# surrealdb/surrealdb

Measured on NVIDIA H100. Metric: KNN queries/sec @recall@10=1.0 (exact brute force), higher is better.
Workload: dtype s8 screen + f64 exact

## Files before the change

### surrealdb_b200/csrc/api.cu

```cuda
#include <cmath>

#include <algorithm>
#include <chrono>

#include "internal.cuh"

namespace sdb {

static thread_local char g_err[1024] = "";
void set_error(const char* fmt, ...) {
  va_list ap;
  va_start(ap, fmt);
  vsnprintf(g_err, sizeof(g_err), fmt, ap);
  va_end(ap);
}


static uint32_t pass_ratio(uint32_t nq) {
  static int env = -1;
  if (env < 0) {
    env = 0;
    if (const char* e = getenv("SDB_PASS_RATIO")) {
      const int v = atoi(e);
      if (v >= 2 && v <= 64) env = v;
// ... 698 lines not shown
      }
    }
  }
  if (lane == 0) out_count[q] = n_out;
}

sdb_status topk_merge_launch(Ctx* ctx, uint32_t n_lists, uint32_t nq, uint32_t k, const uint64_t* d_rows,
                             const double* d_dist, const uint32_t* d_counts, uint64_t stride_rows, uint64_t stride_dist,
                             uint64_t stride_counts, uint64_t* d_out_rows, double* d_out_dist, uint32_t* d_out_count,
                             cudaStream_t st) {
  if (!stride_rows) stride_rows = (uint64_t)nq * k;
  if (!stride_dist) stride_dist = (uint64_t)nq * k;
  if (!stride_counts) stride_counts = nq;
  if (n_lists <= 32) {
    topk_kway_merge_kernel<<<(nq + 3) / 4, 128, 0, st>>>(n_lists, nq, k, d_rows, d_dist, d_counts, stride_rows, stride_dist,
                                                       stride_counts, d_out_rows, d_out_dist, d_out_count);
    count_launch(ctx);
    SDB_CUDA(cudaGetLastError());
    return SDB_OK;
  }
  uint32_t p2 = 1;
  while (p2 < n_lists * k) p2 <<= 1;
  const size_t smem = (size_t)p2 * 24;
  if (smem > 200 * 1024) {
    set_error("merge of %u lists x k=%u exceeds the shared-memory sorter", n_lists, k);
    return SDB_EUNSUPPORTED;
  }
  const uint32_t threads = p2 >= 1024 ? 1024 : (p2 < 64 ? 64 : p2);
  topk_merge_kernel<<<nq, threads, smem, st>>>(n_lists, nq, k, d_rows, d_dist, d_counts, stride_rows, stride_dist,
                                               stride_counts, d_out_rows, d_out_dist, d_out_count);
  count_launch(ctx);
  SDB_CUDA(cudaGetLastError());
  return SDB_OK;
}

}

using namespace sdb;

extern "C" {

const char* sdb_last_error(void) { return g_err; }
const char* sdb_version(void) { return "sdbgpu 0.1.0 (sm_90a)"; }

sdb_status sdb_ctx_create(int device, sdb_ctx** out) {
  if (!out) return SDB_EINVAL;
  *out = nullptr;
  int n = 0;
  cudaError_t e = cudaGetDeviceCount(&n);
  if (e != cudaSuccess || n == 0) {
    set_error("no CUDA device available (%s); this library has no CPU fallback", cudaGetErrorString(e));
    return SDB_ECUDA;
  }
  if (device < 0 || device >= n) {
    set_error("device %d out of range (0..%d)", device, n - 1);
    return SDB_EINVAL;
  }
  cudaDeviceProp prop;
  SDB_CUDA(cudaGetDeviceProperties(&prop, device));
  if (prop.major != 9 || prop.minor != 0) {
    set_error("device %d is sm_%d%d; this library ships sm_90a code only", device, prop.major, prop.minor);
    return SDB_ECUDA;
  }
  SDB_CUDA(cudaSetDevice(device));
  sdb_ctx* c = new sdb_ctx();
  c->device = device;
  c->sm_count = prop.multiProcessorCount;
  {
    int least = 0, greatest = 0;
    if (cudaDeviceGetStreamPriorityRange(&least, &greatest) == cudaSuccess) c->prio_high = greatest;
  }
  SDB_CUDA(cudaStreamCreateWithFlags(&c->stream, cudaStreamNonBlocking));
  SDB_CUDA(cudaStreamCreateWithFlags(&c->stream2, cudaStreamNonBlocking));
  SDB_CUDA(cudaStreamCreateWithFlags(&c->copy_stream, cudaStreamNonBlocking));
  {
    int* hc = nullptr;
    SDB_CUDA(cudaHostAlloc(&hc, sizeof(int), cudaHostAllocMapped));
    *hc = 0;
    c->h_cancel = hc;
    SDB_CUDA(cudaMalloc(&c->d_cancel, sizeof(int)));
    SDB_CUDA(cudaMemset(c->d_cancel, 0, sizeof(int)));
    SDB_CUDA(cudaStreamCreateWithFlags(&c->cancel_stream, cudaStreamNonBlocking));
  }
  SDB_TRY(screen_tc_init_device());
  SDB_TRY(candidates_init_device());
  SDB_TRY(exact_init_device());
  SDB_CUDA(cudaFuncSetAttribute(topk_merge_kernel, cudaFuncAttributeMaxDynamicSharedMemorySize, 200 * 1024));
  {
    cudaMemPool_t pool;
    if (cudaDeviceGetDefaultMemPool(&pool, device) == cudaSuccess) {
      uint64_t thr = ~0ull;
      cudaMemPoolSetAttribute(pool, cudaMemPoolAttrReleaseThreshold, &thr);
    }
  }
  *out = c;
  return SDB_OK;
}
void sdb_ctx_destroy(sdb_ctx* c) {
  if (!c) return;
  cudaSetDevice(c->device);
  comm_destroy(c);
  if (c->stream) cudaStreamDestroy(c->stream);
  if (c->stream2) cudaStreamDestroy(c->stream2);
  if (c->copy_stream) cudaStreamDestroy(c->copy_stream);
  if (c->h_stage) cudaFreeHost(c->h_stage);
  if (c->h_cancel) cudaFreeHost((void*)c->h_cancel);
  if (c->d_cancel) cudaFree(c->d_cancel);
  if (c->cancel_stream) cudaStreamDestroy(c->cancel_stream);
  delete c;
}
static void push_cancel_word(sdb_ctx* c) {
  if (!c->d_cancel || !c->cancel_stream) return;
  if (cudaSetDevice(c->device) != cudaSuccess) return;
  cudaMemcpyAsync(c->d_cancel, (const void*)c->h_cancel, sizeof(int), cudaMemcpyHostToDevice, c->cancel_stream);
  cudaStreamSynchronize(c->cancel_stream);
}
void sdb_ctx_cancel(sdb_ctx* c) {
  if (!c || !c->h_cancel) return;
  *c->h_cancel = 1;
  push_cancel_word(c);
}
void sdb_ctx_cancel_reset(sdb_ctx* c) {
  if (!c || !c->h_cancel) return;
  *c->h_cancel = 0;
  push_cancel_word(c);
}
uint64_t sdb_ctx_kernel_launches(const sdb_ctx* c) { return c ? c->launches : 0; }
void* sdb_ctx_stream(const sdb_ctx* c) { return c ? (void*)c->stream : nullptr; }
void* sdb_pinned_alloc(size_t bytes) {
  void* p = nullptr;
  if (cudaHostAlloc(&p, bytes, cudaHostAllocDefault) != cudaSuccess) {
    set_error("cudaHostAlloc(%zu) failed", bytes);
    return nullptr;
  }
  return p;
}
void sdb_pinned_free(void* p) {
  if (p) cudaFreeHost(p);
}
void sdb_free(void* p) { free(p); }

sdb_status sdb_corpus_create(sdb_ctx* ctx, uint32_t dim, sdb_dtype dt, sdb_metric m, uint64_t cap, sdb_corpus** out) {
  if (!ctx || !out || dim == 0 || dim > 65535 || cap == 0 || cap >= 0xFFFFFFF0ull) {
    set_error("sdb_corpus_create: bad argument (dim 1..65535, 0 < capacity < 2^32)");
    return SDB_EINVAL;
  }
  const bool screenable = m == SDB_COSINE || m == SDB_EUCLIDEAN;
  if ((int)m < 0 || (int)m > (int)SDB_PEARSON) {
    set_error("unknown metric %d", (int)m);
    return SDB_EINVAL;
  }
  if (dt != SDB_F32 && dt != SDB_F64) return SDB_EINVAL;
  SDB_CUDA(cudaSetDevice(ctx->device));
  sdb_corpus* c = new sdb_corpus();
  c->ctx = ctx;
  c->dim = dim;
  c->dim_pad = (dim + 63) / 64 * 64;
  c->dim_pad8 = (dim + 127) / 128 * 128;
  c->dtype = dt;
  c->metric = m;
  c->cap = cap;
  const size_t esz = dt == SDB_F32 ? 4 : 8;
  const uint64_t cap_pad = (cap + TILE_ROWS - 1) / TILE_ROWS * TILE_ROWS;
  cudaError_t e = cudaMalloc(&c->d_rows, esz * cap * dim);
  if (e == cudaSuccess) e = cudaMalloc(&c->d_mag, sizeof(double) * cap);
  if (e == cudaSuccess) e = cudaMalloc(&c->d_snorm, sizeof(float) * cap_pad);
  if (e == cudaSuccess && dt == SDB_F32 && screenable) e = cudaMalloc(&c->d_bf16, sizeof(__nv_bfloat16) * cap_pad * c->dim_pad);
// ... 564 lines not shown
```

### surrealdb_b200/csrc/internal.cuh

```cuda
#pragma once
#include <cuda_bf16.h>
#include <cuda_runtime.h>

#include <cstdarg>
#include <cstdint>
#include <cstdio>
#include <cstdlib>
#include <cstring>
#include <mutex>
#include <vector>

#include "../../include/sdbgpu.h"

namespace sdb {

void set_error(const char* fmt, ...);

#define SDB_CUDA(call)                                                                      \
  do {                                                                                      \
    cudaError_t e__ = (call);                                                               \
    if (e__ != cudaSuccess) {                                                               \
      ::sdb::set_error("%s:%d: %s -> %s", __FILE__, __LINE__, #call, cudaGetErrorString(e__)); \
      return SDB_ECUDA;                                                                     \
    }                                                                                       \
// ... 15 lines not shown
#else
  memcpy(&b, &d, 8);
#endif
  return b;
}
__host__ __device__ inline uint64_t dist_key(double d) {
  uint64_t b = f64_bits(d);
  if ((b << 1) == 0) b = 0;
  return (b >> 63) ? ~b : (b | 0x8000000000000000ull);
}
__host__ __device__ inline uint32_t f32_key(float f) {
  uint32_t b;
#ifdef __CUDA_ARCH__
  asm volatile("mov.b32 %0, %1;" : "=r"(b) : "f"(f));
#else
  memcpy(&b, &f, 4);
#endif
  return (b >> 31) ? ~b : (b | 0x80000000u);
}

constexpr uint32_t HIST_BINS = 256;
constexpr uint32_t PROBE_TILES_MAX = 64;
constexpr uint32_t PROBE_STRIDE = PROBE_TILES_MAX * 8;
struct HistParam {
  float lo;
  float inv_w0;
  float w0;
  float margin;
};
__host__ __device__ inline uint32_t hist_bin(const HistParam& p, float score) {
  float t = (score - p.lo) * p.inv_w0 + 1.0f;
  t = t >= 1.0f ? t : 1.0f;
  uint32_t b;
#ifdef __CUDA_ARCH__
  b = (__float_as_uint(t) - 0x3F800000u) >> 19;
#else
  uint32_t u;
  memcpy(&u, &t, 4);
  b = (u - 0x3F800000u) >> 19;
#endif
  return b < HIST_BINS - 1 ? b : HIST_BINS - 1;
}
__host__ __device__ inline double hist_edge(const HistParam& p, uint32_t b) {
  const uint32_t u = 0x3F800000u + (b << 19);
  float t;
#ifdef __CUDA_ARCH__
  t = __uint_as_float(u);
#else
  memcpy(&t, &u, 4);
#endif
  return (double)p.lo + (double)p.w0 * ((double)t - 1.0);
}

struct PassDesc {
  uint32_t stride;
  uint32_t excl;
  uint32_t count;
  uint32_t perm;
};
__host__ __device__ inline uint32_t pass_tile(const PassDesc& p, uint32_t w) {
  if (p.perm) w = (uint32_t)(((uint64_t)w * p.perm) % p.count);
  uint32_t i = p.excl ? (w / (p.excl - 1)) * p.excl + (w % (p.excl - 1)) + 1 : w;
  return i * p.stride;
}

struct Comm;

struct Ctx {
  int device = 0;
  int sm_count = 132;
  cudaStream_t stream = nullptr;
  cudaStream_t stream2 = nullptr;
  cudaStream_t copy_stream = nullptr;
  uint64_t launches = 0;
  std::mutex mu;
  void* encode_tiled = nullptr;
  void* h_stage = nullptr;
  size_t h_stage_bytes = 0;
  Comm* comm = nullptr;
  volatile int* h_cancel = nullptr;
  int* d_cancel = nullptr;
  cudaStream_t cancel_stream = nullptr;
  int prio_high = 0;
  cudaEvent_t trace_epoch = nullptr;
  double trace_host0 = 0.0;
};
inline bool ctx_cancelled(const Ctx* ctx) { return ctx->h_cancel && *ctx->h_cancel != 0; }

sdb_status screen_tc_init_device();
sdb_status candidates_init_device();
sdb_status exact_init_device();
void comm_destroy(Ctx* ctx);
void comm_corpus_released(struct Corpus* c);
int comm_size(const Ctx* ctx);
int comm_rank(const Ctx* ctx);
sdb_status comm_allreduce_sum(Ctx* ctx, void* d_buf, size_t count, int elem_bytes, cudaStream_t st);

struct Cand {
  float score;
  uint32_t row;
};

struct Ticket {
  bool busy = false;
  uint32_t id = 0;
  const double* d_queries = nullptr;
  uint32_t nq = 0, k = 0;
  uint64_t row_base = 0;
  uint64_t *d_out_rows = nullptr, *h_out_rows = nullptr;
  double *d_out_dist = nullptr, *h_out_dist = nullptr;
  uint32_t *d_out_count = nullptr, *h_out_count = nullptr;
  const volatile int* cancel = nullptr;
  cudaStream_t stream = nullptr;
  int set = 0;
  int screen = 0;
  uint32_t rung = 0, n_rungs = 0, n_batch_rungs = 0, n_repaired = 0;
  uint32_t n_passes = 0;
  uint64_t launches0 = 0;
  cudaEvent_t ev_begin = nullptr, ev_screen0 = nullptr, ev_screen1 = nullptr, ev_end = nullptr;
  uint32_t* h_flags = nullptr;
  uint32_t* h_qflags = nullptr;
  uint32_t* h_stat = nullptr;
  uint32_t h_cap = 0;
  double* d_in_q = nullptr;
  uint64_t* d_res_rows = nullptr;
  double* d_res_dist = nullptr;
  uint32_t* d_res_count = nullptr;
  size_t in_cap = 0, res_cap = 0, res_cap_q = 0;
  cudaEvent_t ev_h2d = nullptr, ev_out = nullptr;
  cudaEvent_t ev_main = nullptr;
  bool wait_h2d = false;
  std::vector<std::pair<const char*, cudaEvent_t>> trace;
};
constexpr int N_TICKETS = 4;
bool trace_enabled();
void trace_mark(Ctx* ctx, Ticket& t, const char* name, cudaStream_t st);
void trace_dump(Ctx* ctx, Ticket& t);
void trace_host(Ctx* ctx, uint32_t ticket, const char* name);

struct Scratch {
  uint32_t sc_nq = 0, sc_cap = 0;
  double* d_q64 = nullptr;
  float* d_q32 = nullptr;
  __nv_bfloat16* d_qbf16 = nullptr;
  double* d_qmag = nullptr;
  uint32_t* d_qflags = nullptr;
  float* d_qbferr = nullptr;
  int8_t* d_q8 = nullptr;
  float* d_q8scale = nullptr;
  float* d_q8err = nullptr;
  Cand* d_sub = nullptr;
  uint32_t* d_sub_cnt = nullptr;
  uint32_t sub_slots = 0, sub_cap = 0, last_slots = 0;
  float* d_bscale = nullptr;
  float* d_beps = nullptr;
  float* d_margin = nullptr;
  float* d_margin2 = nullptr;
  float* d_beps2 = nullptr;
  float* d_tau2 = nullptr;
  float* d_qlow = nullptr;
  float* d_qcap = nullptr;
  HistParam* d_hparam = nullptr;
  uint32_t* d_hist = nullptr;
  float* d_probe = nullptr;
  float* d_tau = nullptr;
  Cand* d_cand = nullptr;
  uint32_t* d_cand_cnt = nullptr;
  uint32_t* d_flags = nullptr;
  uint32_t* d_stat = nullptr;
  uint64_t* d_rr_key = nullptr;
  double* d_rr_dist = nullptr;
  uint32_t* d_rr_row = nullptr;
// ... 110 lines not shown
```

### surrealdb_b200/csrc/screen_tc.cu

```cuda
#include <cuda.h>

#include <type_traits>

#include "internal.cuh"

namespace sdb {

namespace tc {
constexpr uint32_t BLOCK_M = 128;
constexpr uint32_t BLOCK_N = 256;
constexpr uint32_t BLOCK_K = 64;
constexpr uint32_t WG_M = 64;
constexpr uint32_t STAGES = 4;
constexpr uint32_t A_BYTES = BLOCK_M * BLOCK_K * 2;
constexpr uint32_t B_BYTES = BLOCK_N * BLOCK_K * 2;
constexpr uint32_t STAGE_BYTES = A_BYTES + B_BYTES;
constexpr uint32_t CONS_WARPS = 8;
constexpr uint32_t PROD_WARP = CONS_WARPS;
constexpr uint32_t THREADS = (CONS_WARPS + 2) * 32;
constexpr uint32_t MAX_MBLOCKS = 16;
constexpr uint32_t SUBCAP = 16;
constexpr uint32_t SMEM_BYTES = STAGES * STAGE_BYTES + 2 * BLOCK_N * 4 + 256 + MAX_MBLOCKS * 256 * 4 + 1024;
static_assert(BLOCK_N == TILE_ROWS, "screen tile must match the pass schedule tile");
static_assert(SMEM_BYTES <= 227 * 1024, "screen CTA must fit the shared memory of one SM");

__device__ __forceinline__ uint32_t smem_u32(const void* p) { return (uint32_t)__cvta_generic_to_shared(p); }

__device__ __forceinline__ uint32_t item_mb(uint32_t w, uint32_t n_mb) { return (w % n_mb + w / n_mb) % n_mb; }

__device__ __forceinline__ void mbar_init(uint32_t bar, uint32_t count) {
  asm volatile("mbarrier.init.shared::cta.b64 [%0], %1;" ::"r"(bar), "r"(count) : "memory");
}
__device__ __forceinline__ void mbar_expect_tx(uint32_t bar, uint32_t bytes) {
  asm volatile("mbarrier.arrive.expect_tx.shared::cta.b64 _, [%0], %1;" ::"r"(bar), "r"(bytes) : "memory");
}
__device__ __forceinline__ void mbar_arrive(uint32_t bar) {
  asm volatile("mbarrier.arrive.shared::cta.b64 _, [%0];" ::"r"(bar) : "memory");
}
__device__ __forceinline__ void mbar_wait(uint32_t bar, uint32_t parity) {
  uint32_t ok;
  do {
    asm volatile(
        "{\n\t.reg .pred p;\n\t"
        "mbarrier.try_wait.parity.shared::cta.b64 p, [%1], %2;\n\t"
        "selp.u32 %0, 1, 0, p;\n\t}"
        : "=r"(ok)
        : "r"(bar), "r"(parity)
        : "memory");
  } while (!ok);
}
__device__ __forceinline__ void tma_load_2d(uint32_t dst, const CUtensorMap* map, uint32_t c0, uint32_t c1, uint32_t bar) {
  asm volatile(
      "cp.async.bulk.tensor.2d.shared::cluster.global.tile.mbarrier::complete_tx::bytes [%0], [%1, {%2, %3}], [%4];"
      ::"r"(dst), "l"(map), "r"(c0), "r"(c1), "r"(bar)
      : "memory");
}

#define SDB_WG_REGS                                                                                   \
  "{%0, %1, %2, %3, %4, %5, %6, %7, %8, %9, %10, %11, %12, %13, %14, %15, "                           \
  "%16, %17, %18, %19, %20, %21, %22, %23, %24, %25, %26, %27, %28, %29, %30, %31, "                  \
  "%32, %33, %34, %35, %36, %37, %38, %39, %40, %41, %42, %43, %44, %45, %46, %47, "                  \
  "%48, %49, %50, %51, %52, %53, %54, %55, %56, %57, %58, %59, %60, %61, %62, %63, "                  \
  "%64, %65, %66, %67, %68, %69, %70, %71, %72, %73, %74, %75, %76, %77, %78, %79, "                  \
  "%80, %81, %82, %83, %84, %85, %86, %87, %88, %89, %90, %91, %92, %93, %94, %95, "                  \
  "%96, %97, %98, %99, %100, %101, %102, %103, %104, %105, %106, %107, %108, %109, %110, %111, "      \
  "%112, %113, %114, %115, %116, %117, %118, %119, %120, %121, %122, %123, %124, %125, %126, %127}"
#define SDB_WG8(C, i) C(d[i]), C(d[i + 1]), C(d[i + 2]), C(d[i + 3]), C(d[i + 4]), C(d[i + 5]), C(d[i + 6]), C(d[i + 7])
#define SDB_WG128(C)                                                                                     \
  SDB_WG8(C, 0), SDB_WG8(C, 8), SDB_WG8(C, 16), SDB_WG8(C, 24), SDB_WG8(C, 32), SDB_WG8(C, 40), SDB_WG8(C, 48), \
      SDB_WG8(C, 56), SDB_WG8(C, 64), SDB_WG8(C, 72), SDB_WG8(C, 80), SDB_WG8(C, 88), SDB_WG8(C, 96),             \
      SDB_WG8(C, 104), SDB_WG8(C, 112), SDB_WG8(C, 120)

__device__ __forceinline__ void wgmma_bf16(float (&d)[128], uint64_t a_desc, uint64_t b_desc, uint32_t acc) {
  asm volatile(
      "{\n\t.reg .pred p;\n\t"
      "setp.ne.b32 p, %130, 0;\n\t"
      "wgmma.mma_async.sync.aligned.m64n256k16.f32.bf16.bf16 " SDB_WG_REGS ", %128, %129, p, 1, 1, 0, 0;\n\t}"
      : SDB_WG128("+f")
      : "l"(a_desc), "l"(b_desc), "r"(acc));
}
__device__ __forceinline__ void wgmma_i8(uint32_t (&d)[128], uint64_t a_desc, uint64_t b_desc, uint32_t acc) {
  asm volatile(
      "{\n\t.reg .pred p;\n\t"
      "setp.ne.b32 p, %130, 0;\n\t"
      "wgmma.mma_async.sync.aligned.m64n256k32.s32.s8.s8 " SDB_WG_REGS ", %128, %129, p;\n\t}"
      : SDB_WG128("+r")
      : "l"(a_desc), "l"(b_desc), "r"(acc));
}
__device__ __forceinline__ void acc_fence(float (&d)[128]) {
#pragma unroll
  for (int i = 0; i < 128; i++) asm volatile("" : "+f"(d[i])::"memory");
}
__device__ __forceinline__ void acc_fence(uint32_t (&d)[128]) {
#pragma unroll
  for (int i = 0; i < 128; i++) asm volatile("" : "+r"(d[i])::"memory");
}
#undef SDB_WG128
#undef SDB_WG8
#undef SDB_WG_REGS
__device__ __forceinline__ void wgmma_fence() { asm volatile("wgmma.fence.sync.aligned;" ::: "memory"); }
__device__ __forceinline__ void wgmma_commit() { asm volatile("wgmma.commit_group.sync.aligned;" ::: "memory"); }
template <int N>
__device__ __forceinline__ void wgmma_wait() {
  asm volatile("wgmma.wait_group.sync.aligned %0;" ::"n"(N) : "memory");
}
__device__ __forceinline__ uint64_t make_desc(uint32_t saddr) {
  uint64_t d = 0;
  d |= (uint64_t)((saddr >> 4) & 0x3FFF);
  d |= (uint64_t)1 << 16;
  d |= (uint64_t)(1024 >> 4) << 32;
  d |= (uint64_t)1 << 62;
  return d;
}

template <typename Acc>
__device__ __forceinline__ Acc acc_at(const Acc (&acc)[128], int i, int t) {
  return acc[4 * (t >> 1) + 2 * i + (t & 1)];
}
__device__ __forceinline__ uint32_t fragment_col(int t, uint32_t col_l) { return 8 * (t >> 1) + col_l + (t & 1); }
template <typename Acc>
__device__ __forceinline__ Acc acc_at_dyn(const Acc (&acc)[128], int i, int t) {
  Acc v = acc[2 * i];
#pragma unroll
  for (int u = 1; u < 64; u++) v = u == t ? acc_at(acc, i, u) : v;
  return v;
}


template <int MODE>
__device__ __forceinline__ void append_survivor(float score, uint32_t q, uint32_t row, uint32_t col, uint32_t row0,
                                                float2 hpv, uint32_t* s_cnt_mb, Cand* __restrict__ cand,
                                                uint32_t* __restrict__ cand_cnt, uint32_t cap, Cand* __restrict__ sub,
                                                uint32_t* hist) {
  const uint32_t half = col >> 7;
  const uint32_t pos = atomicAdd(s_cnt_mb + half * BLOCK_M + row, 1u);
  const uint2 cd = make_uint2(__float_as_uint(score), row0 + col);
  const uint32_t n_slots = gridDim.x * 2;
  if (pos < SUBCAP) {
    *reinterpret_cast<uint2*>(sub + ((size_t)q * n_slots + blockIdx.x * 2 + half) * SUBCAP + pos) = cd;
  } else {
    const uint32_t p2 = atomicAdd(cand_cnt + q, 1u);
    if (p2 < cap) *reinterpret_cast<uint2*>(cand + (size_t)q * cap + p2) = cd;
  }
  if (MODE == 2) {
    HistParam hp;
    hp.lo = hpv.x;
    hp.inv_w0 = hpv.y;
    hp.w0 = 0.f;
    hp.margin = 0.f;
    atomicAdd(hist + (size_t)q * HIST_BINS + hist_bin(hp, score), 1u);
  }
}

template <bool COSINE, bool INT8, int MODE>
__global__ void __launch_bounds__(THREADS, 1)
screen_tc_kernel(const __grid_constant__ CUtensorMap map_a, const __grid_constant__ CUtensorMap map_b,
                 const float* __restrict__ snorm, uint32_t k_blocks, uint32_t n_mblocks, uint32_t nq,
                 PassDesc pass, float* tau, Cand* __restrict__ cand,
                 uint32_t* __restrict__ cand_cnt, uint32_t cap, Cand* __restrict__ sub, uint32_t* __restrict__ sub_cnt,
                 uint32_t k, const HistParam* __restrict__ hparam, uint32_t* hist, float* __restrict__ probe,
                 uint32_t probe_stride, uint32_t sleep_min_ns, uint32_t sleep_max_ns) {
  extern __shared__ uint8_t smem_raw[];
  uint8_t* smem = reinterpret_cast<uint8_t*>((reinterpret_cast<uintptr_t>(smem_raw) + 1023) & ~uintptr_t(1023));
  uint8_t* smem_a = smem;
  uint8_t* smem_b = smem + STAGES * A_BYTES;
  float* s_snorm = reinterpret_cast<float*>(smem + STAGES * STAGE_BYTES);
  uint64_t* bars = reinterpret_cast<uint64_t*>(s_snorm + 2 * BLOCK_N);
  uint64_t* full_bar = bars;
  uint64_t* empty_bar = bars + STAGES;
  uint32_t* s_done = reinterpret_cast<uint32_t*>(bars + 2 * STAGES);
  uint32_t* s_cnt = reinterpret_cast<uint32_t*>(reinterpret_cast<uint8_t*>(bars) + 256);

  const uint32_t warp = threadIdx.x >> 5, lane = threadIdx.x & 31;
  const uint32_t n_items = pass.count * n_mblocks;

  if (threadIdx.x == 0) {
    asm volatile("prefetch.tensormap [%0];" ::"l"(&map_a) : "memory");
    asm volatile("prefetch.tensormap [%0];" ::"l"(&map_b) : "memory");
    for (uint32_t s = 0; s < STAGES; s++) {
      mbar_init(smem_u32(&full_bar[s]), 1);
      mbar_init(smem_u32(&empty_bar[s]), CONS_WARPS);
    }
    asm volatile("fence.mbarrier_init.release.cluster;" ::: "memory");
    *s_done = 0;
  }
  for (uint32_t i = threadIdx.x; i < n_mblocks * 256; i += blockDim.x) s_cnt[i] = 0;
  __syncthreads();

  if (warp == PROD_WARP) {
    if (lane == 0) {
      uint32_t it = 0;
      for (uint32_t w = blockIdx.x; w < n_items; w += gridDim.x) {
        const uint32_t tile = pass_tile(pass, w / n_mblocks);
        const uint32_t mb = item_mb(w, n_mblocks);
        for (uint32_t kb = 0; kb < k_blocks; kb++, it++) {
          const uint32_t s = it % STAGES, ph = (it / STAGES) & 1;
          mbar_wait(smem_u32(&empty_bar[s]), ph ^ 1);
          const uint32_t fb = smem_u32(&full_bar[s]);
          mbar_expect_tx(fb, STAGE_BYTES);
          tma_load_2d(smem_u32(smem_a + s * A_BYTES), &map_a, kb * (INT8 ? 2 * BLOCK_K : BLOCK_K), mb * BLOCK_M, fb);
          tma_load_2d(smem_u32(smem_b + s * B_BYTES), &map_b, kb * (INT8 ? 2 * BLOCK_K : BLOCK_K), tile * BLOCK_N, fb);
        }
      }
    }
    __syncwarp();
  } else if (warp < CONS_WARPS) {
    const uint32_t ct = threadIdx.x;
    const uint32_t g = warp >> 2;
    const uint32_t row_base = g * WG_M + (warp & 3) * 16 + (lane >> 2);
    const uint32_t col_l = 2 * (lane & 3);
    constexpr bool pass0 = MODE == 0;
    using Acc = typename std::conditional<INT8, uint32_t, float>::type;
    Acc acc[128];
    uint32_t it = 0, j = 0;
    for (uint32_t w = blockIdx.x; w < n_items; w += gridDim.x, j++) {
      const uint32_t tidx = w / n_mblocks;
      const uint32_t tile = pass_tile(pass, tidx);
      const uint32_t mb = item_mb(w, n_mblocks);
      const uint32_t row0 = tile * BLOCK_N;
      float my_tau[2];
      float2 my_hp[2];
#pragma unroll
      for (int i = 0; i < 2; i++) {
        const uint32_t q = mb * BLOCK_M + row_base + 8 * i;
        my_tau[i] = __int_as_float(0x7f800000);
        my_hp[i] = make_float2(0.f, 0.f);
        if (q < nq) {
          my_tau[i] = __ldcg(tau + q);
          if (MODE == 2) my_hp[i] = __ldg(reinterpret_cast<const float2*>(hparam + q));
        }
      }
      float* sn = s_snorm + (j & 1) * BLOCK_N;
      if (!INT8 || MODE == 3) {
        sn[ct] = __ldg(snorm + row0 + ct);
        asm volatile("bar.sync 1, 256;" ::: "memory");
      }

      const uint32_t a_off = g * (WG_M * 128);
      for (uint32_t kb = 0; kb < k_blocks; kb++, it++) {
        const uint32_t s = it % STAGES, ph = (it / STAGES) & 1;
        mbar_wait(smem_u32(&full_bar[s]), ph);
        const uint64_t da = make_desc(smem_u32(smem_a + s * A_BYTES + a_off));
        const uint64_t db = make_desc(smem_u32(smem_b + s * B_BYTES));
        wgmma_fence();
        acc_fence(acc);
#pragma unroll
        for (uint32_t kk = 0; kk < 4; kk++) {
          if constexpr (INT8) wgmma_i8(acc, da + 2 * kk, db + 2 * kk, (kb | kk) != 0);
          else wgmma_bf16(acc, da + 2 * kk, db + 2 * kk, (kb | kk) != 0);
        }
        wgmma_commit();
        acc_fence(acc);
        if (kb > 0) {
          wgmma_wait<1>();
          if (lane == 0) mbar_arrive(smem_u32(&empty_bar[(it - 1) % STAGES]));
        }
      }
      wgmma_wait<0>();
      acc_fence(acc);
      if (lane == 0) mbar_arrive(smem_u32(&empty_bar[(it - 1) % STAGES]));

      if constexpr (!INT8) {
#pragma unroll
        for (int jj = 0; jj < 32; jj++) {
          const float2 n2 = *reinterpret_cast<const float2*>(sn + 8 * jj + col_l);
#pragma unroll
          for (int i = 0; i < 2; i++) {
            float& a0 = acc[4 * jj + 2 * i];
            float& a1 = acc[4 * jj + 2 * i + 1];
            a0 = COSINE ? a0 * n2.x : fmaf(2.f, a0, -n2.x);
            a1 = COSINE ? a1 * n2.y : fmaf(2.f, a1, -n2.y);
          }
        }
      }
#pragma unroll
      for (int i = 0; i < 2; i++) {
        const uint32_t row = row_base + 8 * i;
        const uint32_t q = mb * BLOCK_M + row;
        if (MODE == 3) {
#pragma unroll
          for (int h = 0; h < 8; h++) {
            float m = __int_as_float(0xff800000);
#pragma unroll
            for (int jj = 4 * h; jj < 4 * h + 4; jj++) {
#pragma unroll
              for (int c = 0; c < 2; c++) {
                if constexpr (INT8) {
                  const float snv = sn[8 * jj + col_l + c];
                  if (snv == snv) m = fmaxf(m, __int2float_rd((int)acc[4 * jj + 2 * i + c]));
                } else {
                  m = fmaxf(m, acc[4 * jj + 2 * i + c]);
                }
              }
            }
            m = fmaxf(m, __shfl_xor_sync(0xffffffffu, m, 1));
            m = fmaxf(m, __shfl_xor_sync(0xffffffffu, m, 2));
            if ((lane & 3) == 0 && q < nq) probe[(size_t)q * probe_stride + tidx * 8 + h] = m;
          }
        } else if (pass0) {
          if (q < nq) {
            Cand* my_cand = cand + (size_t)q * cap + (size_t)tidx * BLOCK_N;
#pragma unroll
            for (int jj = 0; jj < 32; jj++) {
              const uint32_t col = 8 * jj + col_l;
              float s0, s1;
              if constexpr (INT8) {
                s0 = __int2float_rn((int)acc[4 * jj + 2 * i]);
                s1 = __int2float_rn((int)acc[4 * jj + 2 * i + 1]);
              } else {
                s0 = acc[4 * jj + 2 * i];
                s1 = acc[4 * jj + 2 * i + 1];
              }
              *reinterpret_cast<uint2*>(my_cand + col) = make_uint2(__float_as_uint(s0), row0 + col);
              *reinterpret_cast<uint2*>(my_cand + col + 1) = make_uint2(__float_as_uint(s1), row0 + col + 1);
            }
          }
        } else {
          uint32_t* s_cnt_mb = s_cnt + mb * 256;
          if constexpr (INT8) {
            const float ct_ = ceilf(my_tau[i]);
            const int tau_i = ct_ >= 2147483520.f ? 0x7fffffff : (ct_ <= -2147483520.f ? (int)0x80000000 : (int)ct_);
            int m = (int)0x80000000;
#pragma unroll
            for (int jj = 0; jj < 32; jj++) m = max(m, max((int)acc[4 * jj + 2 * i], (int)acc[4 * jj + 2 * i + 1]));
            if (m >= tau_i) {
              uint64_t hits = 0;
#pragma unroll
              for (int t = 0; t < 64; t++)
                if ((int)acc_at(acc, i, t) >= tau_i) hits |= 1ull << t;
              while (hits) {
                const int t = __ffsll((long long)hits) - 1;
                hits &= hits - 1;
                const int v = (int)acc_at_dyn(acc, i, t);
                const uint32_t col = fragment_col(t, col_l);
                if (v != 0 || __ldg(snorm + row0 + col) == __ldg(snorm + row0 + col))
                  append_survivor<MODE>(__int2float_rn(v), q, row, col, row0, my_hp[i], s_cnt_mb, cand, cand_cnt,
                                        cap, sub, hist);
              }
            }
          } else {
            float m = __int_as_float(0xff800000);
#pragma unroll
            for (int jj = 0; jj < 32; jj++) m = fmaxf(m, fmaxf(acc[4 * jj + 2 * i], acc[4 * jj + 2 * i + 1]));
            if (m >= my_tau[i]) {
#pragma unroll
              for (int jj = 0; jj < 32; jj++) {
#pragma unroll
                for (int c = 0; c < 2; c++) {
                  const float v = acc[4 * jj + 2 * i + c];
                  if (v >= my_tau[i])
                    append_survivor<MODE>(v, q, row, 8 * jj + col_l + c, row0, my_hp[i], s_cnt_mb, cand, cand_cnt,
                                          cap, sub, hist);
                }
              }
            }
          }
        }
      }
    }
    if (MODE == 1 || MODE == 2) {
      asm volatile("bar.sync 1, 256;" ::: "memory");
      const uint32_t n_slots = gridDim.x * 2;
      const uint32_t half = ct / BLOCK_M, row = ct % BLOCK_M;
      for (uint32_t mb = 0; mb < n_mblocks; mb++) {
        const uint32_t qq = mb * BLOCK_M + row;
        if (qq < nq) sub_cnt[(size_t)qq * n_slots + blockIdx.x * 2 + half] = s_cnt[mb * 256 + half * BLOCK_M + row];
      }
    }
    __syncwarp();
    if (lane == 0) atomicAdd(s_done, 1u);
  } else {
    if (MODE == 2) {
      volatile uint32_t* done = s_done;
      const uint32_t stride = gridDim.x;
      uint32_t n_own = nq > blockIdx.x ? (nq - blockIdx.x + stride - 1) / stride : 0;
      if (n_own > 32) n_own = 32;
      float my_tau = __int_as_float(0xff800000);
      if (lane < n_own) my_tau = __ldcg(tau + blockIdx.x + lane * stride);
      uint32_t sleep_ns = sleep_min_ns;
      while (*done < CONS_WARPS) {
        bool any = false;
        for (uint32_t j = 0; j < n_own; j++) {
          const uint32_t q = blockIdx.x + j * stride;
          const uint4* hq = reinterpret_cast<const uint4*>(hist + (size_t)q * HIST_BINS) + lane * 2;
          const uint4 ha = __ldcg(hq), hb = __ldcg(hq + 1);
          const uint32_t c[8] = {ha.x, ha.y, ha.z, ha.w, hb.x, hb.y, hb.z, hb.w};
          uint32_t sum = 0;
#pragma unroll
          for (int i = 0; i < 8; i++) sum += c[i];
          uint32_t incl = sum;
#pragma unroll
          for (int o = 1; o < 32; o <<= 1) {
            const uint32_t t = __shfl_down_sync(0xffffffffu, incl, o);
            if (lane + o < 32) incl += t;
          }
          const uint32_t above = incl - sum;
          const bool mine = above < k && k <= incl;
          const uint32_t who = __ballot_sync(0xffffffffu, mine);
          if (who == 0) continue;
          uint32_t bstar = 0;
          if (mine) {
            uint32_t acc = above;
#pragma unroll
            for (int i = 7; i >= 0; i--) {
              acc += c[i];
              if (acc >= k) {
                bstar = lane * 8 + i;
                break;
              }
            }
          }
          bstar = __shfl_sync(0xffffffffu, bstar, __ffs(who) - 1);
          const float4 hv = __ldg(reinterpret_cast<const float4*>(hparam + q));
          HistParam hp;
          hp.lo = hv.x;
          hp.inv_w0 = hv.y;
          hp.w0 = hv.z;
          hp.margin = hv.w;
          const double e0 = hist_edge(hp, bstar), e1 = hist_edge(hp, bstar + 1);
          const float tn = __double2float_rd(e0 - (double)hp.margin - 0.02 * (e1 - e0) - 2e-6 * fabs(e0));
          const float told = __shfl_sync(0xffffffffu, my_tau, j);
          if (tn > told) {
            if (lane == j) my_tau = tn;
            if (lane == 0) __stcg(tau + q, tn);
            any = true;
          }
        }
        sleep_ns = any ? sleep_min_ns : (sleep_ns * 2 < sleep_max_ns ? sleep_ns * 2 : sleep_max_ns);
        __nanosleep(sleep_ns);
      }
    }
  }
  __syncthreads();
}
}

typedef CUresult (*EncodeTiledFn)(CUtensorMap*, CUtensorMapDataType, cuuint32_t, void*, const cuuint64_t*,
                                  const cuuint64_t*, const cuuint32_t*, const cuuint32_t*, CUtensorMapInterleave,
                                  CUtensorMapSwizzle, CUtensorMapL2promotion, CUtensorMapFloatOOBfill);

static EncodeTiledFn get_encode(Ctx* ctx) {
  if (!ctx->encode_tiled) {
    void* fn = nullptr;
    cudaDriverEntryPointQueryResult qres;
    if (cudaGetDriverEntryPoint("cuTensorMapEncodeTiled", &fn, cudaEnableDefault, &qres) != cudaSuccess ||
        qres != cudaDriverEntryPointSuccess)
      fn = nullptr;
    ctx->encode_tiled = fn;
  }
  return reinterpret_cast<EncodeTiledFn>(ctx->encode_tiled);
}

static sdb_status make_map(Ctx* ctx, CUtensorMap* map, const void* base, uint64_t rows, uint32_t dim_pad,
                           uint32_t box_rows, bool stream_once, bool int8 = false) {
  EncodeTiledFn enc = get_encode(ctx);
  if (!enc) {
    set_error("cuTensorMapEncodeTiled driver entry point not available");
    return SDB_ECUDA;
  }
  cuuint64_t gdim[2] = {dim_pad, rows};
  cuuint64_t gstride[1] = {(cuuint64_t)dim_pad * (int8 ? 1 : 2)};
  cuuint32_t box[2] = {int8 ? 2 * tc::BLOCK_K : tc::BLOCK_K, box_rows};
  cuuint32_t estr[2] = {1, 1};
  CUresult r = enc(map, int8 ? CU_TENSOR_MAP_DATA_TYPE_UINT8 : CU_TENSOR_MAP_DATA_TYPE_BFLOAT16, 2, const_cast<void*>(base), gdim, gstride, box, estr,
                   CU_TENSOR_MAP_INTERLEAVE_NONE, CU_TENSOR_MAP_SWIZZLE_128B,
                   stream_once ? CU_TENSOR_MAP_L2_PROMOTION_L2_256B : CU_TENSOR_MAP_L2_PROMOTION_L2_128B,
                   CU_TENSOR_MAP_FLOAT_OOB_FILL_NONE);
  if (r != CUDA_SUCCESS) {
    set_error("cuTensorMapEncodeTiled failed (%d)", (int)r);
    return SDB_ECUDA;
  }
  return SDB_OK;
}

bool screen_tc_available() { return true; }

sdb_status screen_tc_init_device() {
#define SET_SMEM(COS, I8, MODE) \
  SDB_CUDA(cudaFuncSetAttribute(tc::screen_tc_kernel<COS, I8, MODE>, cudaFuncAttributeMaxDynamicSharedMemorySize, (int)tc::SMEM_BYTES))
  SET_SMEM(true, false, 0); SET_SMEM(true, false, 1); SET_SMEM(true, false, 2); SET_SMEM(true, false, 3);
  SET_SMEM(false, false, 0); SET_SMEM(false, false, 1); SET_SMEM(false, false, 2); SET_SMEM(false, false, 3);
  SET_SMEM(true, true, 0); SET_SMEM(true, true, 1); SET_SMEM(true, true, 2); SET_SMEM(true, true, 3);
#undef SET_SMEM
  return SDB_OK;
}

sdb_status screen_tc_pass(Corpus* c, uint32_t nq, uint32_t k, const PassDesc& p, bool int8, int mode, cudaStream_t st) {
  if (p.count == 0) return SDB_OK;
  Ctx* ctx = c->ctx;
  if (int8 ? (!c->d_i8 || c->metric != SDB_COSINE) : !c->d_bf16) {
    set_error("tensor-core screen: the %s screen copy is not available for this corpus", int8 ? "int8 (cosine only)" : "bf16");
    return SDB_EUNSUPPORTED;
  }
  const uint64_t n_pad = (c->n + TILE_ROWS - 1) / TILE_ROWS * TILE_ROWS;
  uint32_t sleep_min = 512, sleep_max = 8192;
  if (const char* e = getenv("SDB_REFINE_SLEEP_MIN")) sleep_min = (uint32_t)atoi(e);
  if (const char* e = getenv("SDB_REFINE_SLEEP_MAX")) sleep_max = (uint32_t)atoi(e);
  if (sleep_min < 32) sleep_min = 32;
  if (sleep_max < sleep_min) sleep_max = sleep_min;
  CUtensorMap map_b;
  if (int8) SDB_TRY(make_map(ctx, &map_b, c->d_i8, n_pad, c->dim_pad8, tc::BLOCK_N, true, true));
  else SDB_TRY(make_map(ctx, &map_b, c->d_bf16, n_pad, c->dim_pad, tc::BLOCK_N, true));
  const uint32_t k_blocks = int8 ? c->dim_pad8 / (2 * tc::BLOCK_K) : c->dim_pad / tc::BLOCK_K;
  const uint32_t chunk_q = tc::MAX_MBLOCKS * tc::BLOCK_M;
  uint32_t grid = (uint32_t)ctx->sm_count;
  {
    const uint32_t nq0 = nq < chunk_q ? nq : chunk_q;
    const uint64_t items0 = (uint64_t)p.count * ((nq0 + tc::BLOCK_M - 1) / tc::BLOCK_M);
    if (grid > items0) grid = (uint32_t)items0;
  }
  if (mode == 3 && p.count * 8 > PROBE_STRIDE) {
    set_error("screen_tc_pass: probe of %u tiles exceeds the probe buffer", p.count);
    return SDB_EINVAL;
  }
  if (mode != 3) c->last_slots = grid * 2;
  const uint32_t slots = grid * 2;
  for (uint32_t q0 = 0; q0 < nq; q0 += chunk_q) {
    const uint32_t nqc = nq - q0 < chunk_q ? nq - q0 : chunk_q;
    const uint32_t nq_pad = (nqc + tc::BLOCK_M - 1) / tc::BLOCK_M * tc::BLOCK_M;
    const uint32_t n_mblocks = nq_pad / tc::BLOCK_M;
    CUtensorMap map_a;
    if (int8) SDB_TRY(make_map(ctx, &map_a, c->d_q8 + (size_t)q0 * c->dim_pad8, nq_pad, c->dim_pad8, tc::BLOCK_M, false, true));
    else SDB_TRY(make_map(ctx, &map_a, c->d_qbf16 + (size_t)q0 * c->dim_pad, nq_pad, c->dim_pad, tc::BLOCK_M, false));
    float* tau = c->d_tau + q0;
    Cand* cand = c->d_cand + (size_t)q0 * c->sc_cap;
    uint32_t* ccnt = c->d_cand_cnt + q0;
    Cand* sub = c->d_sub + (size_t)q0 * slots * tc::SUBCAP;
    uint32_t* scnt = c->d_sub_cnt + (size_t)q0 * slots;
    const HistParam* hp = c->d_hparam + q0;
    uint32_t* hist = c->d_hist + (size_t)q0 * HIST_BINS;
    cudaLaunchConfig_t cfg = {};
    cfg.gridDim = dim3(grid);
    cfg.blockDim = dim3(tc::THREADS);
    cfg.dynamicSmemBytes = tc::SMEM_BYTES;
    cfg.stream = st;
    cudaLaunchAttribute attr[1];
    attr[0].id = cudaLaunchAttributePriority;
    attr[0].val.priority = ctx->prio_high;
    cfg.attrs = attr;
    cfg.numAttrs = 1;
    float* probe_ptr = c->d_probe + (size_t)q0 * PROBE_STRIDE;
    const uint32_t probe_stride = PROBE_STRIDE, cap_arg = c->sc_cap;
    const float* snorm_arg = c->d_snorm;
#define LAUNCH_TC1(COS, I8, MODE)                                                                                    \
  SDB_CUDA(cudaLaunchKernelEx(&cfg, tc::screen_tc_kernel<COS, I8, MODE>, map_a, map_b, snorm_arg, k_blocks, n_mblocks, \
                              nqc, p, tau, cand, ccnt, cap_arg, sub, scnt, k, hp, hist, probe_ptr, probe_stride,       \
                              sleep_min, sleep_max))
#define LAUNCH_TC(COS, I8)                   \
  do {                                       \
    if (mode == 0) LAUNCH_TC1(COS, I8, 0);   \
    else if (mode == 1) LAUNCH_TC1(COS, I8, 1); \
    else if (mode == 2) LAUNCH_TC1(COS, I8, 2); \
    else LAUNCH_TC1(COS, I8, 3);             \
  } while (0)
    if (int8) LAUNCH_TC(true, true);
    else if (c->metric == SDB_COSINE) LAUNCH_TC(true, false);
    else LAUNCH_TC(false, false);
#undef LAUNCH_TC
#undef LAUNCH_TC1
    count_launch(ctx);
  }
  if (mode == 0) {
    SDB_TRY(cand_set_count(c, nq, p.count * TILE_ROWS, st));
    c->last_slots = 0;
  }
  SDB_CUDA(cudaGetLastError());
  return SDB_OK;
}

}
```

Baseline: 58460.

## Add drain warp ring for int8 survivors and 2-CTA multicast corpus loads

In int8 screen modes 1 and 2, consumer warps now push threshold survivors into a shared-memory ring that a dedicated drain warp processes. This takes the serial survivor append out of the tensor-core consumer loop. Separately, in mode 2 with an even number of query blocks, CTAs are paired into clusters of two. Each CTA TMA-multicasts half of the corpus tile to both, halving global B-tile traffic. The costs are an extra warp, ring backpressure spins, cross-CTA barrier arrivals, and a grid that may shrink to cluster occupancy.

```diff
diff --git a/surrealdb_b200/csrc/api.cu b/surrealdb_b200/csrc/api.cu
--- a/surrealdb_b200/csrc/api.cu
+++ b/surrealdb_b200/csrc/api.cu
@@ -804,7 +804,7 @@
     SDB_CUDA(cudaMemset(c->d_cancel, 0, sizeof(int)));
     SDB_CUDA(cudaStreamCreateWithFlags(&c->cancel_stream, cudaStreamNonBlocking));
   }
-  SDB_TRY(screen_tc_init_device());
+  SDB_TRY(screen_tc_init_device(c));
   SDB_TRY(candidates_init_device());
   SDB_TRY(exact_init_device());
   SDB_CUDA(cudaFuncSetAttribute(topk_merge_kernel, cudaFuncAttributeMaxDynamicSharedMemorySize, 200 * 1024));
diff --git a/surrealdb_b200/csrc/internal.cuh b/surrealdb_b200/csrc/internal.cuh
--- a/surrealdb_b200/csrc/internal.cuh
+++ b/surrealdb_b200/csrc/internal.cuh
@@ -121,12 +121,13 @@
   int* d_cancel = nullptr;
   cudaStream_t cancel_stream = nullptr;
   int prio_high = 0;
+  int tc_pair_ctas = 0;
   cudaEvent_t trace_epoch = nullptr;
   double trace_host0 = 0.0;
 };
 inline bool ctx_cancelled(const Ctx* ctx) { return ctx->h_cancel && *ctx->h_cancel != 0; }
 
-sdb_status screen_tc_init_device();
+sdb_status screen_tc_init_device(Ctx* ctx);
 sdb_status candidates_init_device();
 sdb_status exact_init_device();
 void comm_destroy(Ctx* ctx);
diff --git a/surrealdb_b200/csrc/screen_tc.cu b/surrealdb_b200/csrc/screen_tc.cu
--- a/surrealdb_b200/csrc/screen_tc.cu
+++ b/surrealdb_b200/csrc/screen_tc.cu
@@ -17,12 +17,19 @@
 constexpr uint32_t STAGE_BYTES = A_BYTES + B_BYTES;
 constexpr uint32_t CONS_WARPS = 8;
 constexpr uint32_t PROD_WARP = CONS_WARPS;
-constexpr uint32_t THREADS = (CONS_WARPS + 2) * 32;
+constexpr uint32_t DRAIN_WARP = CONS_WARPS + 2;
 constexpr uint32_t MAX_MBLOCKS = 16;
 constexpr uint32_t SUBCAP = 16;
 constexpr uint32_t SMEM_BYTES = STAGES * STAGE_BYTES + 2 * BLOCK_N * 4 + 256 + MAX_MBLOCKS * 256 * 4 + 1024;
 static_assert(BLOCK_N == TILE_ROWS, "screen tile must match the pass schedule tile");
 static_assert(SMEM_BYTES <= 227 * 1024, "screen CTA must fit the shared memory of one SM");
+constexpr uint32_t RING = 128;
+static_assert(3 * RING * 4 <= 2 * BLOCK_N * 4, "the survivor ring must fit the screening-norm buffers");
+static_assert(MAX_MBLOCKS * BLOCK_M <= 0x10000 && RING <= 32 * 1024, "ring tags: 16-bit query and sequence fields");
+template <bool INT8, int MODE>
+constexpr bool has_drain() { return INT8 && (MODE == 1 || MODE == 2); }
+template <bool INT8, int MODE>
+constexpr uint32_t threads() { return (CONS_WARPS + (has_drain<INT8, MODE>() ? 3 : 2)) * 32; }
 
 __device__ __forceinline__ uint32_t smem_u32(const void* p) { return (uint32_t)__cvta_generic_to_shared(p); }
 
@@ -54,6 +61,27 @@
       "cp.async.bulk.tensor.2d.shared::cluster.global.tile.mbarrier::complete_tx::bytes [%0], [%1, {%2, %3}], [%4];"
       ::"r"(dst), "l"(map), "r"(c0), "r"(c1), "r"(bar)
       : "memory");
+}
+__device__ __forceinline__ void tma_load_2d_pair(uint32_t dst, const CUtensorMap* map, uint32_t c0, uint32_t c1,
+                                                 uint32_t bar) {
+  asm volatile(
+      "cp.async.bulk.tensor.2d.shared::cluster.global.tile.mbarrier::complete_tx::bytes.multicast::cluster"
+      " [%0], [%1, {%2, %3}], [%4], %5;"
+      ::"r"(dst), "l"(map), "r"(c0), "r"(c1), "r"(bar), "h"((uint16_t)0x3)
+      : "memory");
+}
+__device__ __forceinline__ void mbar_arrive_cta(uint32_t bar, uint32_t rank) {
+  uint32_t remote;
+  asm volatile("mapa.shared::cluster.u32 %0, %1, %2;" : "=r"(remote) : "r"(bar), "r"(rank));
+  asm volatile("mbarrier.arrive.shared::cluster.b64 _, [%0];" ::"r"(remote) : "memory");
+}
+__device__ __forceinline__ uint32_t cluster_ctarank() {
+  uint32_t r;
+  asm volatile("mov.u32 %0, %%cluster_ctarank;" : "=r"(r));
+  return r;
+}
+__device__ __forceinline__ void cluster_sync() {
+  asm volatile("barrier.cluster.arrive.release.aligned;\n\tbarrier.cluster.wait.acquire.aligned;" ::: "memory");
 }
 
 #define SDB_WG_REGS                                                                                   \
@@ -125,6 +153,8 @@
   for (int u = 1; u < 64; u++) v = u == t ? acc_at(acc, i, u) : v;
   return v;
 }
+__device__ __forceinline__ uint32_t ld_volatile(const uint32_t* p) { return *reinterpret_cast<const volatile uint32_t*>(p); }
+__device__ __forceinline__ void st_volatile(uint32_t* p, uint32_t v) { *reinterpret_cast<volatile uint32_t*>(p) = v; }
 
 
 template <int MODE>
@@ -152,14 +182,42 @@
   }
 }
 
+__device__ __forceinline__ void push_survivors(const uint32_t (&acc)[128], int i, uint64_t hits, uint32_t q,
+                                               uint32_t row0, uint32_t col_l, uint32_t lane, uint32_t* r_val,
+                                               uint32_t* r_row, uint32_t* r_tag, uint32_t* s_ring_tail,
+                                               const uint32_t* s_ring_head) {
+  const uint32_t total = __reduce_add_sync(0xffffffffu, (uint32_t)__popcll(hits));
+  if (total == 0) return;
+  uint32_t base = 0;
+  if (lane == 0) base = atomicAdd(s_ring_tail, total);
+  base = __shfl_sync(0xffffffffu, base, 0);
+  const uint32_t lt = (1u << lane) - 1;
+  for (uint32_t off = 0; off < total;) {
+    const uint32_t act = __ballot_sync(0xffffffffu, hits != 0);
+    const uint32_t e = base + off + __popc(act & lt);
+    off += __popc(act);
+    while ((int)(base + off - RING - ld_volatile(s_ring_head)) > 0) {
+    }
+    if (hits) {
+      const int t = __ffsll((long long)hits) - 1;
+      hits &= hits - 1;
+      const uint32_t slot = e % RING;
+      r_val[slot] = acc_at_dyn(acc, i, t);
+      r_row[slot] = row0 + fragment_col(t, col_l);
+      __threadfence_block();
+      st_volatile(r_tag + slot, e << 16 | q);
+    }
+  }
+}
+
 template <bool COSINE, bool INT8, int MODE>
-__global__ void __launch_bounds__(THREADS, 1)
+__global__ void __launch_bounds__(threads<INT8, MODE>(), 1)
 screen_tc_kernel(const __grid_constant__ CUtensorMap map_a, const __grid_constant__ CUtensorMap map_b,
                  const float* __restrict__ snorm, uint32_t k_blocks, uint32_t n_mblocks, uint32_t nq,
                  PassDesc pass, float* tau, Cand* __restrict__ cand,
                  uint32_t* __restrict__ cand_cnt, uint32_t cap, Cand* __restrict__ sub, uint32_t* __restrict__ sub_cnt,
                  uint32_t k, const HistParam* __restrict__ hparam, uint32_t* hist, float* __restrict__ probe,
-                 uint32_t probe_stride, uint32_t sleep_min_ns, uint32_t sleep_max_ns) {
+                 uint32_t probe_stride, uint32_t sleep_min_ns, uint32_t sleep_max_ns, uint32_t pair) {
   extern __shared__ uint8_t smem_raw[];
   uint8_t* smem = reinterpret_cast<uint8_t*>((reinterpret_cast<uintptr_t>(smem_raw) + 1023) & ~uintptr_t(1023));
   uint8_t* smem_a = smem;
@@ -169,37 +227,58 @@
   uint64_t* full_bar = bars;
   uint64_t* empty_bar = bars + STAGES;
   uint32_t* s_done = reinterpret_cast<uint32_t*>(bars + 2 * STAGES);
+  uint32_t* s_ring_tail = s_done + 1;
+  uint32_t* s_ring_head = s_done + 2;
   uint32_t* s_cnt = reinterpret_cast<uint32_t*>(reinterpret_cast<uint8_t*>(bars) + 256);
+  uint32_t* r_val = reinterpret_cast<uint32_t*>(s_snorm);
+  uint32_t* r_row = r_val + RING;
+  uint32_t* r_tag = r_row + RING;
+  constexpr bool DRAIN = has_drain<INT8, MODE>();
 
   const uint32_t warp = threadIdx.x >> 5, lane = threadIdx.x & 31;
-  const uint32_t n_items = pass.count * n_mblocks;
-
+  const bool PAIR = INT8 && MODE == 2 && pair != 0;
+  const uint32_t rank = PAIR ? cluster_ctarank() : 0;
+  const uint32_t n_mb = PAIR ? n_mblocks / 2 : n_mblocks;
+  const uint32_t w_first = PAIR ? blockIdx.x / 2 : blockIdx.x, w_step = PAIR ? gridDim.x / 2 : gridDim.x;
+  const uint32_t n_items = pass.count * n_mb;
+
+  if (DRAIN) {
+    for (uint32_t i = threadIdx.x; i < RING; i += blockDim.x) r_tag[i] = 0xFFFF0000u;
+  }
   if (threadIdx.x == 0) {
+    *s_ring_tail = 0;
+    *s_ring_head = 0;
     asm volatile("prefetch.tensormap [%0];" ::"l"(&map_a) : "memory");
     asm volatile("prefetch.tensormap [%0];" ::"l"(&map_b) : "memory");
     for (uint32_t s = 0; s < STAGES; s++) {
       mbar_init(smem_u32(&full_bar[s]), 1);
-      mbar_init(smem_u32(&empty_bar[s]), CONS_WARPS);
+      mbar_init(smem_u32(&empty_bar[s]), PAIR ? 2 * CONS_WARPS : CONS_WARPS);
     }
     asm volatile("fence.mbarrier_init.release.cluster;" ::: "memory");
     *s_done = 0;
   }
   for (uint32_t i = threadIdx.x; i < n_mblocks * 256; i += blockDim.x) s_cnt[i] = 0;
   __syncthreads();
+  if (PAIR) cluster_sync();
 
   if (warp == PROD_WARP) {
     if (lane == 0) {
       uint32_t it = 0;
-      for (uint32_t w = blockIdx.x; w < n_items; w += gridDim.x) {
-        const uint32_t tile = pass_tile(pass, w / n_mblocks);
-        const uint32_t mb = item_mb(w, n_mblocks);
+      for (uint32_t w = w_first; w < n_items; w += w_step) {
+        const uint32_t tile = pass_tile(pass, w / n_mb);
+        const uint32_t mb = PAIR ? 2 * item_mb(w, n_mb) + rank : item_mb(w, n_mb);
         for (uint32_t kb = 0; kb < k_blocks; kb++, it++) {
           const uint32_t s = it % STAGES, ph = (it / STAGES) & 1;
           mbar_wait(smem_u32(&empty_bar[s]), ph ^ 1);
           const uint32_t fb = smem_u32(&full_bar[s]);
+          const uint32_t kc = kb * (INT8 ? 2 * BLOCK_K : BLOCK_K);
           mbar_expect_tx(fb, STAGE_BYTES);
-          tma_load_2d(smem_u32(smem_a + s * A_BYTES), &map_a, kb * (INT8 ? 2 * BLOCK_K : BLOCK_K), mb * BLOCK_M, fb);
-          tma_load_2d(smem_u32(smem_b + s * B_BYTES), &map_b, kb * (INT8 ? 2 * BLOCK_K : BLOCK_K), tile * BLOCK_N, fb);
+          tma_load_2d(smem_u32(smem_a + s * A_BYTES), &map_a, kc, mb * BLOCK_M, fb);
+          if (PAIR)
+            tma_load_2d_pair(smem_u32(smem_b + s * B_BYTES + rank * (B_BYTES / 2)), &map_b, kc,
+                             tile * BLOCK_N + rank * (BLOCK_N / 2), fb);
+          else
+            tma_load_2d(smem_u32(smem_b + s * B_BYTES), &map_b, kc, tile * BLOCK_N, fb);
         }
       }
     }
@@ -213,10 +292,16 @@
     using Acc = typename std::conditional<INT8, uint32_t, float>::type;
     Acc acc[128];
     uint32_t it = 0, j = 0;
-    for (uint32_t w = blockIdx.x; w < n_items; w += gridDim.x, j++) {
-      const uint32_t tidx = w / n_mblocks;
+    auto release = [&](uint32_t s) {
+      if (lane == 0) {
+        mbar_arrive(smem_u32(&empty_bar[s]));
+        if (PAIR) mbar_arrive_cta(smem_u32(&empty_bar[s]), rank ^ 1);
+      }
+    };
+    for (uint32_t w = w_first; w < n_items; w += w_step, j++) {
+      const uint32_t tidx = w / n_mb;
       const uint32_t tile = pass_tile(pass, tidx);
-      const uint32_t mb = item_mb(w, n_mblocks);
+      const uint32_t mb = PAIR ? 2 * item_mb(w, n_mb) + rank : item_mb(w, n_mb);
       const uint32_t row0 = tile * BLOCK_N;
       float my_tau[2];
       float2 my_hp[2];
@@ -253,12 +338,12 @@
         acc_fence(acc);
         if (kb > 0) {
           wgmma_wait<1>();
-          if (lane == 0) mbar_arrive(smem_u32(&empty_bar[(it - 1) % STAGES]));
+          release((it - 1) % STAGES);
         }
       }
       wgmma_wait<0>();
       acc_fence(acc);
-      if (lane == 0) mbar_arrive(smem_u32(&empty_bar[(it - 1) % STAGES]));
+      release((it - 1) % STAGES);
 
       if constexpr (!INT8) {
 #pragma unroll
@@ -323,20 +408,14 @@
             int m = (int)0x80000000;
 #pragma unroll
             for (int jj = 0; jj < 32; jj++) m = max(m, max((int)acc[4 * jj + 2 * i], (int)acc[4 * jj + 2 * i + 1]));
-            if (m >= tau_i) {
+            if (__any_sync(0xffffffffu, m >= tau_i)) {
               uint64_t hits = 0;
-#pragma unroll
-              for (int t = 0; t < 64; t++)
-                if ((int)acc_at(acc, i, t) >= tau_i) hits |= 1ull << t;
-              while (hits) {
-                const int t = __ffsll((long long)hits) - 1;
-                hits &= hits - 1;
-                const int v = (int)acc_at_dyn(acc, i, t);
-                const uint32_t col = fragment_col(t, col_l);
-                if (v != 0 || __ldg(snorm + row0 + col) == __ldg(snorm + row0 + col))
-                  append_survivor<MODE>(__int2float_rn(v), q, row, col, row0, my_hp[i], s_cnt_mb, cand, cand_cnt,
-                                        cap, sub, hist);
+              if (m >= tau_i) {
+#pragma unroll
+                for (int t = 0; t < 64; t++)
+                  if ((int)acc_at(acc, i, t) >= tau_i) hits |= 1ull << t;
               }
+              push_survivors(acc, i, hits, q, row0, col_l, lane, r_val, r_row, r_tag, s_ring_tail, s_ring_head);
             }
           } else {
             float m = __int_as_float(0xff800000);
@@ -358,8 +437,14 @@
         }
       }
     }
+    if (DRAIN) {
+      __syncwarp();
+      __threadfence_block();
+      if (lane == 0) atomicAdd(s_done, 1u);
+    }
     if (MODE == 1 || MODE == 2) {
-      asm volatile("bar.sync 1, 256;" ::: "memory");
+      if (DRAIN) asm volatile("bar.sync 2, 288;" ::: "memory");
+      else asm volatile("bar.sync 1, 256;" ::: "memory");
       const uint32_t n_slots = gridDim.x * 2;
       const uint32_t half = ct / BLOCK_M, row = ct % BLOCK_M;
       for (uint32_t mb = 0; mb < n_mblocks; mb++) {
@@ -368,7 +453,43 @@
       }
     }
     __syncwarp();
-    if (lane == 0) atomicAdd(s_done, 1u);
+    if (!DRAIN && lane == 0) atomicAdd(s_done, 1u);
+  } else if (warp == DRAIN_WARP) {
+    if (DRAIN) {
+      uint32_t head = 0;
+      for (;;) {
+        const uint32_t e = head + lane, slot = e % RING;
+        const uint32_t tag = ld_volatile(r_tag + slot);
+        const uint32_t ready = __ballot_sync(0xffffffffu, (tag >> 16) == (e & 0xFFFFu));
+        const uint32_t n = ready == 0xffffffffu ? 32 : __ffs(~ready) - 1;
+        if (n == 0) {
+          uint32_t fin = 0;
+          if (lane == 0 && ld_volatile(s_done) == CONS_WARPS) {
+            __threadfence_block();
+            fin = ld_volatile(s_ring_tail) == head;
+          }
+          if (__shfl_sync(0xffffffffu, fin, 0)) break;
+          __nanosleep(32);
+          continue;
+        }
+        __threadfence_block();
+        if (lane < n) {
+          const int v = (int)r_val[slot];
+          const uint32_t grow = r_row[slot], q = tag & 0xFFFFu;
+          const uint32_t col = grow % BLOCK_N, row = q % BLOCK_M;
+          if (v != 0 || __ldg(snorm + grow) == __ldg(snorm + grow)) {
+            const float2 hpv = MODE == 2 ? __ldg(reinterpret_cast<const float2*>(hparam + q)) : make_float2(0.f, 0.f);
+            append_survivor<MODE>(__int2float_rn(v), q, row, col, grow - col, hpv, s_cnt + q / BLOCK_M * 256, cand,
+                                  cand_cnt, cap, sub, hist);
+          }
+        }
+        __syncwarp();
+        __threadfence_block();
+        head += n;
+        if (lane == 0) st_volatile(s_ring_head, head);
+      }
+      asm volatile("bar.sync 2, 288;" ::: "memory");
+    }
   } else {
     if (MODE == 2) {
       volatile uint32_t* done = s_done;
@@ -432,6 +553,7 @@
     }
   }
   __syncthreads();
+  if (PAIR) cluster_sync();
 }
 }
 
@@ -475,13 +597,27 @@
 
 bool screen_tc_available() { return true; }
 
-sdb_status screen_tc_init_device() {
+sdb_status screen_tc_init_device(Ctx* ctx) {
 #define SET_SMEM(COS, I8, MODE) \
   SDB_CUDA(cudaFuncSetAttribute(tc::screen_tc_kernel<COS, I8, MODE>, cudaFuncAttributeMaxDynamicSharedMemorySize, (int)tc::SMEM_BYTES))
   SET_SMEM(true, false, 0); SET_SMEM(true, false, 1); SET_SMEM(true, false, 2); SET_SMEM(true, false, 3);
   SET_SMEM(false, false, 0); SET_SMEM(false, false, 1); SET_SMEM(false, false, 2); SET_SMEM(false, false, 3);
   SET_SMEM(true, true, 0); SET_SMEM(true, true, 1); SET_SMEM(true, true, 2); SET_SMEM(true, true, 3);
 #undef SET_SMEM
+  cudaLaunchConfig_t cfg = {};
+  cfg.gridDim = dim3((uint32_t)ctx->sm_count & ~1u);
+  cfg.blockDim = dim3(tc::threads<true, 2>());
+  cfg.dynamicSmemBytes = tc::SMEM_BYTES;
+  cudaLaunchAttribute attr[1];
+  attr[0].id = cudaLaunchAttributeClusterDimension;
+  attr[0].val.clusterDim.x = 2;
+  attr[0].val.clusterDim.y = 1;
+  attr[0].val.clusterDim.z = 1;
+  cfg.attrs = attr;
+  cfg.numAttrs = 1;
+  int clusters = 0;
+  SDB_CUDA(cudaOccupancyMaxActiveClusters(&clusters, tc::screen_tc_kernel<true, true, 2>, &cfg));
+  ctx->tc_pair_ctas = 2 * clusters;
   return SDB_OK;
 }
 
@@ -498,17 +634,27 @@
   if (const char* e = getenv("SDB_REFINE_SLEEP_MAX")) sleep_max = (uint32_t)atoi(e);
   if (sleep_min < 32) sleep_min = 32;
   if (sleep_max < sleep_min) sleep_max = sleep_min;
-  CUtensorMap map_b;
-  if (int8) SDB_TRY(make_map(ctx, &map_b, c->d_i8, n_pad, c->dim_pad8, tc::BLOCK_N, true, true));
-  else SDB_TRY(make_map(ctx, &map_b, c->d_bf16, n_pad, c->dim_pad, tc::BLOCK_N, true));
   const uint32_t k_blocks = int8 ? c->dim_pad8 / (2 * tc::BLOCK_K) : c->dim_pad / tc::BLOCK_K;
   const uint32_t chunk_q = tc::MAX_MBLOCKS * tc::BLOCK_M;
+  const uint32_t nq0 = nq < chunk_q ? nq : chunk_q;
+  const uint32_t mb0 = (nq0 + tc::BLOCK_M - 1) / tc::BLOCK_M;
+  const uint32_t mb_last = (nq - (nq - 1) / chunk_q * chunk_q + tc::BLOCK_M - 1) / tc::BLOCK_M;
   uint32_t grid = (uint32_t)ctx->sm_count;
   {
-    const uint32_t nq0 = nq < chunk_q ? nq : chunk_q;
-    const uint64_t items0 = (uint64_t)p.count * ((nq0 + tc::BLOCK_M - 1) / tc::BLOCK_M);
+    const uint64_t items0 = (uint64_t)p.count * mb0;
     if (grid > items0) grid = (uint32_t)items0;
   }
+  uint32_t pair = 0;
+  if (int8 && mode == 2 && mb0 % 2 == 0 && mb_last % 2 == 0) {
+    const uint32_t g2 = (grid < (uint32_t)ctx->tc_pair_ctas ? grid : (uint32_t)ctx->tc_pair_ctas) & ~1u;
+    if (g2 >= 2) {
+      grid = g2;
+      pair = 1;
+    }
+  }
+  CUtensorMap map_b;
+  if (int8) SDB_TRY(make_map(ctx, &map_b, c->d_i8, n_pad, c->dim_pad8, pair ? tc::BLOCK_N / 2 : tc::BLOCK_N, true, true));
+  else SDB_TRY(make_map(ctx, &map_b, c->d_bf16, n_pad, c->dim_pad, tc::BLOCK_N, true));
   if (mode == 3 && p.count * 8 > PROBE_STRIDE) {
     set_error("screen_tc_pass: probe of %u tiles exceeds the probe buffer", p.count);
     return SDB_EINVAL;
@@ -531,21 +677,27 @@
     uint32_t* hist = c->d_hist + (size_t)q0 * HIST_BINS;
     cudaLaunchConfig_t cfg = {};
     cfg.gridDim = dim3(grid);
-    cfg.blockDim = dim3(tc::THREADS);
     cfg.dynamicSmemBytes = tc::SMEM_BYTES;
     cfg.stream = st;
-    cudaLaunchAttribute attr[1];
+    cudaLaunchAttribute attr[2];
     attr[0].id = cudaLaunchAttributePriority;
     attr[0].val.priority = ctx->prio_high;
+    attr[1].id = cudaLaunchAttributeClusterDimension;
+    attr[1].val.clusterDim.x = pair ? 2 : 1;
+    attr[1].val.clusterDim.y = 1;
+    attr[1].val.clusterDim.z = 1;
     cfg.attrs = attr;
-    cfg.numAttrs = 1;
+    cfg.numAttrs = pair ? 2 : 1;
     float* probe_ptr = c->d_probe + (size_t)q0 * PROBE_STRIDE;
     const uint32_t probe_stride = PROBE_STRIDE, cap_arg = c->sc_cap;
     const float* snorm_arg = c->d_snorm;
 #define LAUNCH_TC1(COS, I8, MODE)                                                                                    \
-  SDB_CUDA(cudaLaunchKernelEx(&cfg, tc::screen_tc_kernel<COS, I8, MODE>, map_a, map_b, snorm_arg, k_blocks, n_mblocks, \
-                              nqc, p, tau, cand, ccnt, cap_arg, sub, scnt, k, hp, hist, probe_ptr, probe_stride,       \
-                              sleep_min, sleep_max))
+  do {                                                                                                               \
+    cfg.blockDim = dim3(tc::threads<I8, MODE>());                                                                    \
+    SDB_CUDA(cudaLaunchKernelEx(&cfg, tc::screen_tc_kernel<COS, I8, MODE>, map_a, map_b, snorm_arg, k_blocks,        \
+                                n_mblocks, nqc, p, tau, cand, ccnt, cap_arg, sub, scnt, k, hp, hist, probe_ptr,      \
+                                probe_stride, sleep_min, sleep_max, pair));                                          \
+  } while (0)
 #define LAUNCH_TC(COS, I8)                   \
   do {                                       \
     if (mode == 0) LAUNCH_TC1(COS, I8, 0);   \
```

Result: faster. 62830, median of 6 (+7.5%).
